# huggingface/tokenizers

Hardware: NVIDIA H100
Metric: encode_batch input throughput (higher is better)
Workload: dtype u8

## Files before the change

### __graft_entry__.py

```python
import os, subprocess, sys

ROOT = os.path.dirname(os.path.abspath(__file__))
if ROOT not in sys.path:
    sys.path.insert(0, ROOT)


def build():
    subprocess.check_call(["make", "-s", "-C", os.path.join(ROOT, "tokenizers_b200", "csrc")])
    subprocess.check_call(["make", "-s", "-C", os.path.join(ROOT, "oracle")])
    sys.path.insert(0, os.path.join(ROOT, "tools"))
    import corpus
    corpus.build()
    subprocess.check_call(["g++", "-O2", "-std=c++17", "-shared", "-fPIC", "-o", os.path.join(ROOT, "tests", "native", "libpretok_emul.so"),
                           os.path.join(ROOT, "tests", "native", "pretok_emul.cpp")])
    subprocess.check_call(["g++", "-O2", "-std=c++17", "-I/usr/local/cuda/include", "-Wno-attributes", "-shared", "-fPIC", "-o",
                           os.path.join(ROOT, "tests", "native", "libadded_emul.so"), os.path.join(ROOT, "tests", "native", "added_emul.cpp")])
    subprocess.check_call(["g++", "-O2", "-std=c++17", "-I/usr/local/cuda/include", "-Wno-attributes", "-shared", "-fPIC", "-o",
                           os.path.join(ROOT, "tests", "native", "libdense_emul.so"), os.path.join(ROOT, "tests", "native", "dense_emul.cpp")])
    subprocess.check_call(["g++", "-O2", "-std=c++17", "-I/usr/local/cuda/include", "-Wno-attributes", "-shared", "-fPIC", "-o",
                           os.path.join(ROOT, "tests", "native", "liboverflow_emul.so"), os.path.join(ROOT, "tests", "native", "overflow_emul.cpp")])
    subprocess.check_call(["g++", "-O2", "-std=c++17", "-I/usr/local/cuda/include", "-Wno-attributes", "-shared", "-fPIC", "-o",
                           os.path.join(ROOT, "tests", "native", "libmeta_emul.so"), os.path.join(ROOT, "tests", "native", "meta_emul.cpp")])
    subprocess.check_call(["g++", "-O2", "-std=c++17", "-I/usr/local/cuda/include", "-Wno-attributes", "-shared", "-fPIC", "-include", "cuda_runtime.h", "-o",
                           os.path.join(ROOT, "tests", "native", "libnorm_emul.so"), os.path.join(ROOT, "tests", "native", "norm_emul.cpp"),
                           "-x", "c++", os.path.join(ROOT, "tokenizers_b200", "csrc", "host_tables.cu")])
    import tokenizers_b200
    from tokenizers_b200 import _lib
    _lib.lib()


def smoke():
    import gzip
    import numpy as np
    sys.path.insert(0, os.path.join(ROOT, "tools"))
    import corpus
    from tokenizers_b200 import Tokenizer
    from oracle import oracle as orc
    for name, kind in (("gpt2_style", 2), ("llama3_style", 2), ("wordpiece", 4)):
        js = gzip.open(os.path.join(ROOT, "assets", name + ".json.gz")).read().decode("utf-8")
        tok = Tokenizer.from_str(js, device=0)
        data, off = corpus.generate(kind, 7, 0, 2000)
        be = tok.encode_batch_csr(data, off)
        ids, offs, wid, rp = orc.Oracle(js).encode_batch_csr(data, off)
        assert np.array_equal(be.ids, ids) and np.array_equal(be.offsets, offs) and np.array_equal(be.word_ids, wid) and np.array_equal(be.row_ptr, rp), name
        print(f"smoke {name}: {len(off) - 1} docs, {len(data)} bytes -> {len(ids)} tokens, bit-exact vs oracle")
    import json
    j = json.loads(gzip.open(os.path.join(ROOT, "assets", "wordpiece.json.gz")).read().decode("utf-8"))
    j["normalizer"] = {"type": "BertNormalizer", "clean_text": True, "handle_chinese_chars": True, "strip_accents": None, "lowercase": True}
    j["pre_tokenizer"] = {"type": "BertPreTokenizer"}
    js = json.dumps(j)
    tok = Tokenizer.from_str(js, device=0)
    data, off = corpus.generate(2, 8, 0, 1500)
    be = tok.encode_batch_csr(data, off)
    ids, offs, wid, rp = orc.Oracle(js).encode_batch_csr(data, off)
    assert np.array_equal(be.ids, ids) and np.array_equal(be.offsets, offs) and np.array_equal(be.word_ids, wid) and np.array_equal(be.row_ptr, rp), "bert"
    tok.enable_truncation(32); tok.enable_padding(length=32, pad_id=0)
    dn = tok.encode_batch_dense(data, off, add_special_tokens=False)
    exp = orc.dense_rows(ids, rp, length=32, pad_to_multiple_of=0, max_length=32, pad_id=0, truncate_left=False, pad_left=False, pre=[], post=[])
    assert np.array_equal(dn["input_ids"], exp[0]) and np.array_equal(dn["attention_mask"], exp[1]), "dense"
    print(f"smoke bert_uncased: {len(off) - 1} docs -> {len(ids)} tokens, offsets into the original text and dense [n, 32] rows bit-exact vs oracle")


if __name__ == "__main__":
    build()
    if len(sys.argv) > 1 and sys.argv[1] == "smoke":
        smoke()
```

### tokenizers_b200/csrc/b2t_tables.h

```cpp
#pragma once
#include <stdint.h>

#if defined(__CUDACC__)
#define B2T_HDI __host__ __device__ __forceinline__
#else
#define B2T_HDI inline
#endif

namespace b2t {

constexpr uint32_t EMPTY_KEY = 0xFFFFFFFFu;
constexpr uint64_t NO_MERGE = ~0ull;

B2T_HDI uint32_t pair_hash(uint32_t a, uint32_t b) {
  uint32_t h = a * 0x9E3779B1u ^ (b * 0x85EBCA77u + 0x165667B1u);
  h ^= h >> 15; h *= 0x2C1B3C6Du; h ^= h >> 12;
  return h;
}

struct StrHash {
  uint32_t h1, h2;
};
B2T_HDI void strhash_init(StrHash& s) { s.h1 = 0x811C9DC5u; s.h2 = 0x9747B28Cu; }
B2T_HDI void strhash_byte(StrHash& s, uint32_t b) {
  s.h1 = (s.h1 ^ b) * 0x01000193u;
  s.h2 = (s.h2 + b + 1u) * 0x5BD1E995u; s.h2 ^= s.h2 >> 13;
}
B2T_HDI void strhash_fin(StrHash& s) {
  s.h1 ^= s.h1 >> 16; s.h1 *= 0x7FEB352Du; s.h1 ^= s.h1 >> 15;
  s.h2 ^= s.h2 >> 15; s.h2 *= 0x846CA68Bu; s.h2 ^= s.h2 >> 16;
}

B2T_HDI uint32_t edge_hash(uint32_t node, uint32_t byte) {
  uint32_t h = (node * 256u + byte) * 0x9E3779B1u;
  h ^= h >> 16; h *= 0x85EBCA6Bu; h ^= h >> 13;
  return h;
}

enum { NORM_IDENT = 0u, NORM_REMOVE = 1u, NORM_STRING = 2u, NORM_SURVIVOR = 3u, NORM_MARK_FLAG = 4u, NORM_TAIL_FLAG = 0x80u };
constexpr uint32_t NORM_LEN_MASK = 31u;

B2T_HDI bool norm_mark_neighbour(uint32_t cp, uint32_t e, const uint8_t* ascii) {
  if (cp < 128u) return ascii[cp] == 0xFFu;
  const uint32_t kind = e & 3u;
  return kind == NORM_SURVIVOR || (kind == NORM_REMOVE && (e & NORM_MARK_FLAG) != 0u);
}

struct DeviceTables {
  const uint32_t* byte_to_id;
  const uint4* merge_tbl;
  uint32_t merge_mask;
  const uint4* word_tbl;
  uint32_t word_mask;
  const uint8_t* word_pool;
  int ignore_merges;
  int monotone;
  const uint32_t* tok2_bits;
  const uint32_t* tri_bits;
  const uint4* edge_tbl;
  uint32_t edge_mask;
  uint32_t unk_id;
  uint32_t max_chars;
};

}
```

### tokenizers_b200/csrc/engine.cu

```cuda
#include <cuda_runtime.h>
#include <stdarg.h>
#include <stdio.h>
#include <stdlib.h>
#include <string.h>

#include <algorithm>
#include <atomic>
#include <condition_variable>
#include <memory>
#include <mutex>
#include <string>
#include <vector>

#include "../../include/b2t.h"
#include "added_kernels.cuh"
#include "dense_kernels.cuh"
#include "host_tables.h"
#include "long_kernels.cuh"
#include "model_kernels.cuh"
#include "norm_kernels.cuh"
#include "prefix_kernels.cuh"
#include "pretok_kernels.cuh"

using namespace b2t;
// ... 113 lines not shown
  DevBuf bytes, doc_off;
  DevBuf doc_bits, start_bits, drop_bits, page_sum, page_carry, block_sum, block_carry, page_first_doc, ctl;
  DevBuf ids, offsets, word_ids, row_ptr, row_ptr_local;
  Request req;
  Batch batch;
  bool pending = false;
  DevBuf tmp_ids, tmp_offsets, tmp_word_ids, tile_count, tile_first, tile_lexcl, tile_bsum;
  DevBuf page_long, long_desc, long_desc1, soft_bits, page_soft, lp_id, lp_val, lp_len, lp_plen, lp_aux, lp_out;
  unsigned long long pool_cap = 0;
  DevBuf wcache;
  DevBuf dense_ids, dense_mask, dense_len, dense_type;
  DevBuf dense_off, row_count, row_lexcl, row_bsum, row_base, row_sample;
  DevBuf dense_special, dense_seq, dense_word;
  DevBuf nrm_doc_bits, nrm_pfd, nrm_page_out, nrm_page_chars, nrm_lexcl_o, nrm_bsum_o, nrm_lexcl_c, nrm_bsum_c, nrm_tot, nrm_bytes, nrm_src_char, nrm_doc_off, nrm_doc_char0;
  bool norm_active = false;
  DevBuf cand0, cand1, cand_any, hard_bits, inner_bits, added_bits, added_head, added_pool;
  uint32_t added_cap = 0;
  DevBuf pfx_bytes, pfx_doc_off, pfx_local, pfx_block, prefix_bits, pfx_total;
  cudaStream_t stream = nullptr;
  cudaEvent_t done = nullptr;
  PinBuf h_ctl;
  ~Workspace() {
    if (stream) cudaStreamDestroy(stream);
    if (done) cudaEventDestroy(done);
  }
};

struct b2t_result {
  b2t_engine* eng = nullptr;
  int on_device = 0;
  uint32_t n_docs = 0;
  uint64_t n_tokens = 0;
  const uint32_t* ids = nullptr; const uint32_t* offsets = nullptr; const uint32_t* word_ids = nullptr; const uint64_t* row_ptr = nullptr;
  PinBuf h_ids, h_offsets, h_word_ids, h_row_ptr;
  uint32_t dense_len = 0;
  const uint32_t* dense_ids = nullptr; const uint8_t* dense_mask = nullptr; const uint32_t* row_len = nullptr;
  const uint8_t* type_ids = nullptr;
  uint32_t n_rows = 0;
  const uint32_t* row_sample = nullptr; const uint32_t* dense_off = nullptr;
  const uint8_t* special_mask = nullptr; const int8_t* seq_ids = nullptr; const uint32_t* dense_word = nullptr;
  PinBuf h_dense_ids, h_dense_mask, h_row_len, h_type_ids, h_row_sample, h_dense_off, h_special, h_seq, h_word;
};

constexpr int NSLOT = 3;
constexpr int MAX_KERNEL_RECORDS = 16;

struct b2t_engine {
  int device = 0;
  int model = 0, pretok = 0, add_prefix_space = 0;
  int sm_count = 132;
  int wcache_on = 1;
  DeviceTables dt;
  int monotone = 0;
  DevBuf d_cls, d_byte_to_id, d_merge, d_word, d_pool, d_edge, d_tok2, d_tri;
  int norm_on = 0;
  NormTables nt;
  DevBuf d_nt_blk, d_nt_ent, d_nt_pool, d_nt_ascii;
  int has_added = 0;
  AddedTables at;
  DevBuf d_at_bytes, d_at_off, d_at_id, d_at_flags, d_at_first, d_at_pair, d_cls_rust;
  DevBuf d_trim_vocab, d_trim_added;
  uint32_t n_trim_added = 0;
  int trim_ready = 0, added_both = 0;
  std::mutex mu;
  std::mutex dev_mu;
  std::mutex prof_mu;
  std::condition_variable set_free;
  Workspace dev_ws;
  struct SlotSet { Workspace slot[NSLOT]; bool busy = false; };
  std::vector<std::unique_ptr<SlotSet>> sets;
  cudaStream_t own_stream = nullptr;
  size_t chunk_bytes = 64u << 20;
  std::vector<std::unique_ptr<b2t_result>> pool;
  int profiling = 0;
  int n_rec = 0;
  const char* rec_name[MAX_KERNEL_RECORDS];
  cudaEvent_t rec_ev[MAX_KERNEL_RECORDS + 1];
  bool rec_ev_made = false;
  std::atomic<int> last_launches{0};
  ~b2t_engine() {
    if (rec_ev_made) for (auto& ev : rec_ev) cudaEventDestroy(ev);
    if (own_stream) cudaStreamDestroy(own_stream);
  }
};
constexpr size_t MAX_SLOT_SETS = 4;

template <class T>
static int upload(DevBuf& b, const std::vector<T>& v) {
  size_t bytes = v.size() * sizeof(T);
  int rc = b.ensure(bytes ? bytes : 16);
  if (rc) return rc;
  if (bytes) CU(cudaMemcpy(b.p, v.data(), bytes, cudaMemcpyHostToDevice));
  return B2T_OK;
}

extern "C" int b2t_engine_create(const b2t_config* cfg, b2t_engine** out) {
  if (!cfg || !out) return fail(B2T_ERR_INVALID, "b2t_engine_create: null argument");
  if (cfg->struct_size != sizeof(b2t_config)) return fail(B2T_ERR_INVALID, "b2t_engine_create: struct_size mismatch (%u != %zu)", cfg->struct_size, sizeof(b2t_config));
  *out = nullptr;
  if (cfg->model != B2T_MODEL_BPE && cfg->model != B2T_MODEL_WORDPIECE) return fail(B2T_ERR_UNSUPPORTED, "unsupported model kind %d", cfg->model);
  if (cfg->pretok < 0 || cfg->pretok > 4) return fail(B2T_ERR_UNSUPPORTED, "unsupported pre-tokenizer kind %d", cfg->pretok);
  if (cfg->model == B2T_MODEL_BPE && (cfg->pretok == B2T_PRETOK_WHITESPACE || cfg->pretok == B2T_PRETOK_BERT))
    return fail(B2T_ERR_UNSUPPORTED, "BPE is supported behind the ByteLevel pre-tokenizers only");
  if (cfg->model == B2T_MODEL_WORDPIECE && cfg->pretok != B2T_PRETOK_WHITESPACE && cfg->pretok != B2T_PRETOK_BERT)
    return fail(B2T_ERR_UNSUPPORTED, "WordPiece is supported behind the Whitespace and Bert pre-tokenizers only");
  if ((cfg->bert_normalizer & B2T_NORM_BERT) && cfg->model != B2T_MODEL_WORDPIECE)
    return fail(B2T_ERR_UNSUPPORTED, "BertNormalizer is supported in front of WordPiece pipelines only");
  if (cfg->bert_normalizer & ~(B2T_NORM_BERT | B2T_NORM_CLEAN_TEXT | B2T_NORM_CHINESE_CHARS | B2T_NORM_STRIP_ACCENTS | B2T_NORM_LOWERCASE))
    return fail(B2T_ERR_INVALID, "unknown bits in bert_normalizer");
  if (cfg->add_prefix_space && cfg->pretok != B2T_PRETOK_BYTELEVEL && cfg->pretok != B2T_PRETOK_BYTELEVEL_NOREGEX)
    return fail(B2T_ERR_UNSUPPORTED, "add_prefix_space is only meaningful for a top-level ByteLevel pre-tokenizer");
  if (!cfg->vocab_bytes || !cfg->vocab_off || !cfg->vocab_ids || cfg->n_vocab == 0) return fail(B2T_ERR_INVALID, "empty vocabulary");

  HostTables ht;
  bool vocab_err = false;
  std::string msg = build_host_tables(cfg->model, cfg->pretok, cfg->ignore_merges, cfg->n_vocab, cfg->vocab_bytes, cfg->vocab_off,
                                      cfg->vocab_ids, cfg->n_merges, cfg->merge_bytes, cfg->merge_off, cfg->unk_token,
                                      cfg->continuing_subword_prefix, cfg->max_input_chars_per_word, &ht, &vocab_err);
  if (!msg.empty()) return fail(vocab_err ? B2T_ERR_VOCAB : B2T_ERR_UNSUPPORTED, "%s", msg.c_str());

  int ndev = 0;
  cudaError_t ce = cudaGetDeviceCount(&ndev);
  if (ce != cudaSuccess || ndev == 0)
    return fail(B2T_ERR_CUDA, "no CUDA device available (%s); this engine has no CPU path", cudaGetErrorString(ce));
  int dev = cfg->device;
  if (dev < 0) CU(cudaGetDevice(&dev));
  if (dev >= ndev) return fail(B2T_ERR_INVALID, "device %d out of range (%d devices)", dev, ndev);
  CU(cudaSetDevice(dev));

  std::unique_ptr<b2t_engine, void (*)(b2t_engine*)> e(new b2t_engine(), b2t_engine_destroy);
  e->device = dev; e->model = cfg->model; e->pretok = cfg->pretok; e->add_prefix_space = cfg->add_prefix_space;
  cudaDeviceGetAttribute(&e->sm_count, cudaDevAttrMultiProcessorCount, dev);
  if (const char* wc = getenv("B2T_WCACHE")) e->wcache_on = atoi(wc) != 0;
  if (const char* cb = getenv("B2T_CHUNK_BYTES")) {
    long long v = atoll(cb);
    if (v >= 1024 && v < (1ll << 31)) e->chunk_bytes = (size_t)v;
  }
  int rc = B2T_OK;
  if ((rc = upload(e->d_cls, ht.cls_packed)) || (rc = upload(e->d_byte_to_id, ht.byte_to_id)) || (rc = upload(e->d_merge, ht.merge_tbl)) ||
      (rc = upload(e->d_word, ht.word_tbl)) || (rc = upload(e->d_pool, ht.word_pool)) || (rc = upload(e->d_edge, ht.edge_tbl)) ||
      (rc = upload(e->d_tok2, ht.tok2_bits)) || (rc = upload(e->d_tri, ht.tri_bits)))
    return rc;
  if (cfg->bert_normalizer & B2T_NORM_BERT) {
    NormHost nh;
    build_bert_norm((cfg->bert_normalizer & B2T_NORM_CLEAN_TEXT) != 0, (cfg->bert_normalizer & B2T_NORM_CHINESE_CHARS) != 0,
                    (cfg->bert_normalizer & B2T_NORM_STRIP_ACCENTS) != 0, (cfg->bert_normalizer & B2T_NORM_LOWERCASE) != 0, &nh);
    if (!nh.ok) return fail(B2T_ERR_UNSUPPORTED, "BertNormalizer table: an image exceeds three bytes per input byte");
    if ((rc = upload(e->d_nt_blk, nh.blk)) || (rc = upload(e->d_nt_ent, nh.ent)) || (rc = upload(e->d_nt_pool, nh.pool)) || (rc = upload(e->d_nt_ascii, nh.ascii)))
      return rc;
    e->nt.blk = e->d_nt_blk.as<uint16_t>(); e->nt.ent = e->d_nt_ent.as<uint32_t>(); e->nt.pool = e->d_nt_pool.as<uint8_t>(); e->nt.ascii = e->d_nt_ascii.as<uint8_t>();
    e->norm_on = 1;
  }
  memset(&e->dt, 0, sizeof(e->dt));
  e->dt.byte_to_id = e->d_byte_to_id.as<uint32_t>();
  e->dt.merge_tbl = e->d_merge.as<uint4>();
  e->dt.merge_mask = ht.merge_tbl.empty() ? 0 : (uint32_t)ht.merge_tbl.size() - 1;
  e->dt.word_tbl = e->d_word.as<uint4>();
  e->dt.word_mask = ht.word_tbl.empty() ? 0 : (uint32_t)ht.word_tbl.size() - 1;
  e->dt.word_pool = e->d_pool.as<uint8_t>();
  e->dt.ignore_merges = cfg->ignore_merges ? 1 : 0;
  e->dt.monotone = ht.monotone ? 1 : 0;
  e->dt.tok2_bits = e->d_tok2.as<uint32_t>(); e->dt.tri_bits = e->d_tri.as<uint32_t>();
  e->monotone = e->dt.monotone;
  e->dt.edge_tbl = e->d_edge.as<uint4>();
  e->dt.edge_mask = ht.edge_tbl.empty() ? 0 : (uint32_t)ht.edge_tbl.size() - 1;
  e->dt.unk_id = ht.unk_id;
  e->dt.max_chars = ht.max_chars;
  cudaFuncSetAttribute(model_tile_kernel<MODEL_BPE>, cudaFuncAttributePreferredSharedMemoryCarveout, 86);
  cudaFuncSetAttribute(model_tile_kernel<MODEL_WORDPIECE>, cudaFuncAttributePreferredSharedMemoryCarveout, 86);
  if (cfg->model == B2T_MODEL_BPE) {
    if ((rc = upload(e->d_trim_vocab, vocab_trim_counts(cfg->n_vocab, cfg->vocab_bytes, cfg->vocab_off, cfg->vocab_ids)))) return rc;
    e->trim_ready = 1;
  }
  cudaError_t se = cudaStreamCreateWithFlags(&e->own_stream, cudaStreamNonBlocking);
  if (se != cudaSuccess) return fail(B2T_ERR_CUDA, "cudaStreamCreate failed: %s", cudaGetErrorString(se));
  *out = e.release();
  return B2T_OK;
}

extern "C" void b2t_engine_destroy(b2t_engine* e) {
  if (!e) return;
  cudaSetDevice(e->device);
  cudaDeviceSynchronize();
  delete e;
}

struct ctl_block {
  uint32_t max_row;
  uint32_t err;
  unsigned long long total;
  LongCtl lc;
  uint32_t added_used;
  uint32_t max_all;
  unsigned long long rows;
  uint32_t stride_m;
  uint32_t pad;
};

static int ensure_long_pool(Workspace& ws, unsigned long long bytes) {
  if (bytes <= ws.pool_cap) return B2T_OK;
  unsigned long long cap = bytes + bytes / 4 + 4096;
  int rc;
  if ((rc = ws.lp_id.ensure(cap * 4)) || (rc = ws.lp_val.ensure(cap * 8)) || (rc = ws.lp_len.ensure(cap * 4)) || (rc = ws.lp_plen.ensure(cap * 4)) ||
      (rc = ws.lp_aux.ensure(cap * 4)) || (rc = ws.lp_out.ensure(cap * 16)))
    return rc;
  ws.pool_cap = cap;
  return B2T_OK;
}

template <int KIND>
static void launch_pretok(b2t_engine* e, const uint8_t* d_bytes, int64_t n, Workspace& ws, cudaStream_t st, bool added) {
  const int64_t n_chunks = n / CHUNK + 1;
  const int64_t n_kb = (n_chunks + 31) / 32;
  const int64_t resident = (int64_t)e->sm_count * (KIND == PT_LLAMA3 ? K1_WINDOW_MINBLOCKS : K1_LEAN_MINBLOCKS) * (K1_THREADS / 32);
  int64_t kb = (n_kb + resident * 4 - 1) / (resident * 4);
  kb = std::min<int64_t>(128, std::max<int64_t>(2, (kb + 1) & ~1ll));
  const int64_t n_warps = (n_kb + kb - 1) / kb;
  const int64_t grid = (n_warps + (K1_THREADS / 32) - 1) / (K1_THREADS / 32);
// ... 1137 lines not shown
```

### tokenizers_b200/csrc/host_tables.cu

```cuda
#include "host_tables.h"

#include <string.h>
#include <vector_types.h>

#include <algorithm>

#include "pretok_logic.cuh"
#include "unicode_ranges.inc"
#include "bert_tables.inc"

namespace b2t {

void unicode_class_table(int scheme, uint8_t* out) {
  memset(out, 0, 0x110000);
  auto fill = [&](const uint32_t (*r)[2], uint32_t cnt, uint8_t v) {
    for (uint32_t i = 0; i < cnt; ++i)
      for (uint32_t c = r[i][0]; c <= r[i][1]; ++c) out[c] = v;
  };
  if (scheme == 0) {
    fill(B2T_ONIG_L, B2T_ONIG_L_COUNT, CLS_L);
    fill(B2T_ONIG_N, B2T_ONIG_N_COUNT, CLS_N);
    fill(B2T_ONIG_S, B2T_ONIG_S_COUNT, CLS_S);
  } else if (scheme == 2) {
    memset(out, CLS_L, 0x110000);
// ... 83 lines not shown
            if (!in_ranges(B2T_BERT_MN, B2T_BERT_MN_COUNT, x)) {
              seq.push_back(x);
              kept_mark = kept_mark || in_ranges(B2T_BERT_CCC, B2T_BERT_CCC_COUNT, x);
            }
        }
        if (lowercase) {
          tmp.clear();
          for (uint32_t x : seq) { auto it = low.find(x); if (it == low.end()) tmp.push_back(x); else tmp.insert(tmp.end(), it->second.begin(), it->second.end()); }
          seq.swap(tmp);
        }
        const bool reorders = strip_accents && in_ranges(B2T_BERT_CCC, B2T_BERT_CCC_COUNT, c);
        if (seq.empty()) e = NORM_REMOVE | (reorders || (strip_accents && cleaned) ? NORM_MARK_FLAG : 0u);
        else if (reorders) {
          e = (seq.size() == 1 && seq[0] == c) ? NORM_SURVIVOR : (NORM_SURVIVOR | NORM_MARK_FLAG);
        } else if (!(seq.size() == 1 && seq[0] == c)) {
          img.clear();
          for (uint32_t x : seq) utf8_append(img, x);
          const size_t src_len = c < 0x80 ? 1 : (c < 0x800 ? 2 : (c < 0x10000 ? 3 : 4));
          if (img.size() > 3 * src_len || img.size() > NORM_LEN_MASK) out->ok = false;
          e = NORM_STRING | ((uint32_t)img.size() << 2) | ((uint32_t)out->pool.size() << 8) | (kept_mark ? NORM_TAIL_FLAG : 0u);
          out->pool.insert(out->pool.end(), img.begin(), img.end());
        }
        if (c < 128) out->ascii[c] = seq.empty() ? 0xFF : (uint8_t)seq[0];
      }
      block[c - b0] = e;
      any = any || e != NORM_IDENT;
    }
    if (any) { out->blk[b0 >> 7] = (uint16_t)(out->ent.size() / 128); out->ent.insert(out->ent.end(), block.begin(), block.end()); }
  }
  out->pool.resize(out->pool.size() + 16, 0);
}

static void utf8_append(std::string& s, uint32_t cp) {
  if (cp < 0x80) s.push_back((char)cp);
  else if (cp < 0x800) { s.push_back((char)(0xC0 | (cp >> 6))); s.push_back((char)(0x80 | (cp & 63))); }
  else if (cp < 0x10000) { s.push_back((char)(0xE0 | (cp >> 12))); s.push_back((char)(0x80 | ((cp >> 6) & 63))); s.push_back((char)(0x80 | (cp & 63))); }
  else { s.push_back((char)(0xF0 | (cp >> 18))); s.push_back((char)(0x80 | ((cp >> 12) & 63))); s.push_back((char)(0x80 | ((cp >> 6) & 63))); s.push_back((char)(0x80 | (cp & 63))); }
}

static void bytes_char_table(uint32_t cp_of_byte[256]) {
  uint32_t k = 0;
  for (int b = 0; b < 256; ++b) {
    bool printable = (b >= '!' && b <= '~') || (b >= 0xA1 && b <= 0xAC) || (b >= 0xAE && b <= 0xFF);
    cp_of_byte[b] = printable ? (uint32_t)b : 256u + k++;
  }
}

static uint32_t pow2_at_least(uint64_t x) {
  uint32_t c = 16;
  while (c < x) c <<= 1;
  return c;
}

std::string build_host_tables(int model, int pretok, int ignore_merges, uint32_t n_vocab, const uint8_t* vocab_bytes,
                              const uint32_t* vocab_off, const uint32_t* vocab_ids, uint32_t n_merges,
                              const uint8_t* merge_bytes, const uint32_t* merge_off, const char* unk_token,
                              const char* cont_prefix, uint32_t max_chars, HostTables* out, bool* vocab_err) {
  *vocab_err = false;
  {
    std::vector<uint8_t> cls(0x110000);
    unicode_class_table(pretok == PT_BERT ? 2 : (pretok == PT_WHITESPACE ? 1 : 0), cls.data());
    out->cls_packed.assign(0x110000 / 16, 0u);
    for (uint32_t c = 0; c < 0x110000; ++c) out->cls_packed[c >> 4] |= (uint32_t)cls[c] << ((c & 15) * 2);
  }
  std::unordered_map<std::string, uint32_t> vocab;
  vocab.reserve((size_t)n_vocab * 2);
  for (uint32_t i = 0; i < n_vocab; ++i) {
    if (vocab_ids[i] >= (1u << 20)) return "token ids of 2^20 and above are not supported";
    vocab[std::string((const char*)vocab_bytes + vocab_off[i], vocab_off[i + 1] - vocab_off[i])] = vocab_ids[i];
  }
  out->max_chars = max_chars;

  if (model == 0) {
    uint32_t cp_of_byte[256];
    bytes_char_table(cp_of_byte);
    std::unordered_map<uint32_t, uint8_t> byte_of_cp;
    out->byte_to_id.assign(256, 0);
    for (int b = 0; b < 256; ++b) {
      std::string ch;
      utf8_append(ch, cp_of_byte[b]);
      auto it = vocab.find(ch);
      if (it == vocab.end())
        return "BPE vocab lacks the ByteLevel character of byte " + std::to_string(b) +
               " (the reference would silently drop such bytes; unsupported on device)";
      out->byte_to_id[b] = it->second;
      byte_of_cp[cp_of_byte[b]] = (uint8_t)b;
    }
    uint32_t cap = pow2_at_least((uint64_t)n_merges * 5 / 2 + 16);
    out->merge_tbl.assign(cap, make_uint4(EMPTY_KEY, EMPTY_KEY, EMPTY_KEY, EMPTY_KEY));
    for (uint32_t i = 0; i < n_merges; ++i) {
      std::string a((const char*)merge_bytes + merge_off[2 * i], merge_off[2 * i + 1] - merge_off[2 * i]);
      std::string b((const char*)merge_bytes + merge_off[2 * i + 1], merge_off[2 * i + 2] - merge_off[2 * i + 1]);
      auto ia = vocab.find(a), ib = vocab.find(b), in = vocab.find(a + b);
      if (ia == vocab.end() || ib == vocab.end() || in == vocab.end()) {
        *vocab_err = true;
        return "merge " + std::to_string(i) + ": token out of vocabulary";
      }
      uint32_t h = pair_hash(ia->second, ib->second) & (cap - 1);
      while (true) {
        uint4& e = out->merge_tbl[h];
        if (e.x == EMPTY_KEY || (e.x == ia->second && e.y == ib->second)) {
          e = make_uint4(ia->second, ib->second, i, in->second);
          break;
        }
        h = (h + 1) & (cap - 1);
      }
    }
    {
      std::unordered_map<uint32_t, uint32_t> created;
      bool mono = true;
      uint32_t live = 0;
      for (const uint4& e : out->merge_tbl) {
        if (e.x == EMPTY_KEY) continue;
        ++live;
        auto it = created.find(e.w);
        if (it == created.end() || it->second < e.z) created[e.w] = e.z;
      }
      if (live != n_merges) mono = false;
      for (const uint4& e : out->merge_tbl) {
        if (e.x == EMPTY_KEY) continue;
        auto ia = created.find(e.x), ib = created.find(e.y);
        if ((ia != created.end() && ia->second >= e.z) || (ib != created.end() && ib->second >= e.z)) { mono = false; break; }
      }
      out->monotone = mono;
    }
    {
      out->tok2_bits.assign((1u << 16) / 32, 0u);
      out->tri_bits.assign((1u << 24) / 32, 0u);
      for (uint32_t i = 0; i < n_vocab; ++i) {
        const uint8_t* s = vocab_bytes + vocab_off[i];
        const uint32_t len = vocab_off[i + 1] - vocab_off[i];
        std::vector<uint8_t> raw;
        bool ok = len > 0;
        for (uint32_t p = 0; p < len && ok;) {
          uint32_t b0 = s[p], cp, l;
          if (b0 < 0x80) { cp = b0; l = 1; }
          else if (b0 < 0xE0 && p + 1 < len) { cp = ((b0 & 31u) << 6) | (s[p + 1] & 63u); l = 2; }
          else { ok = false; break; }
          auto it = byte_of_cp.find(cp);
          if (it == byte_of_cp.end()) { ok = false; break; }
          raw.push_back((uint8_t)it->second);
          p += l;
        }
        if (!ok) continue;
        if (raw.size() == 2) { const uint32_t k = raw[0] | ((uint32_t)raw[1] << 8); out->tok2_bits[k >> 5] |= 1u << (k & 31); }
        for (size_t p = 0; p + 2 < raw.size(); ++p) {
          const uint32_t k = raw[p] | ((uint32_t)raw[p + 1] << 8) | ((uint32_t)raw[p + 2] << 16);
          out->tri_bits[k >> 5] |= 1u << (k & 31);
        }
      }
    }
    if (ignore_merges) {
      uint32_t wcap = pow2_at_least((uint64_t)n_vocab * 5 / 2 + 16);
      out->word_tbl.assign(wcap, make_uint4(0, 0, EMPTY_KEY, 0));
      for (uint32_t i = 0; i < n_vocab; ++i) {
        const uint8_t* s = vocab_bytes + vocab_off[i];
        uint32_t len = vocab_off[i + 1] - vocab_off[i];
        std::string raw;
        bool ok = len > 0;
        for (uint32_t p = 0; p < len && ok;) {
          uint32_t b0 = s[p], cp, l;
          if (b0 < 0x80) { cp = b0; l = 1; }
          else if (b0 < 0xE0 && p + 1 < len) { cp = ((b0 & 31u) << 6) | (s[p + 1] & 63u); l = 2; }
          else { ok = false; break; }
          auto it = byte_of_cp.find(cp);
          if (it == byte_of_cp.end()) { ok = false; break; }
          raw.push_back((char)it->second);
          p += l;
        }
        if (!ok) continue;
        StrHash h;
        strhash_init(h);
        for (unsigned char c : raw) strhash_byte(h, c);
        strhash_fin(h);
        uint32_t slot = h.h1 & (wcap - 1);
        while (out->word_tbl[slot].z != EMPTY_KEY) slot = (slot + 1) & (wcap - 1);
        out->word_tbl[slot] = make_uint4(h.h2, (uint32_t)raw.size(), vocab_ids[i], (uint32_t)out->word_pool.size());
        out->word_pool.insert(out->word_pool.end(), raw.begin(), raw.end());
      }
      out->word_pool.resize(out->word_pool.size() + 16, 0);
    }
  } else {
    if (!unk_token) return "WordPiece needs unk_token";
    if ((uint64_t)max_chars * 4 > 416) return "max_input_chars_per_word above 104 is not supported";
    auto iu = vocab.find(unk_token);
    if (iu == vocab.end()) {
      *vocab_err = true;
      return "WordPiece error: Missing [UNK] token from the vocabulary";
    }
    out->unk_id = iu->second;
    std::string prefix = cont_prefix ? cont_prefix : "";
    std::unordered_map<uint64_t, uint32_t> edges;
    std::vector<uint32_t> node_tok(2, EMPTY_KEY);
    auto insert = [&](uint32_t root, const uint8_t* s, uint32_t len, uint32_t id) {
      uint32_t node = root;
      for (uint32_t p = 0; p < len; ++p) {
        uint64_t key = ((uint64_t)node << 8) | s[p];
        auto it = edges.find(key);
        if (it == edges.end()) {
          uint32_t child = (uint32_t)node_tok.size();
          node_tok.push_back(EMPTY_KEY);
          edges.emplace(key, child);
          node = child;
        } else node = it->second;
      }
      node_tok[node] = id;
    };
    for (uint32_t i = 0; i < n_vocab; ++i) {
      const uint8_t* s = vocab_bytes + vocab_off[i];
      uint32_t len = vocab_off[i + 1] - vocab_off[i];
      if (len == 0) continue;
      insert(0, s, len, vocab_ids[i]);
      if (len > prefix.size() && memcmp(s, prefix.data(), prefix.size()) == 0)
        insert(1, s + prefix.size(), len - (uint32_t)prefix.size(), vocab_ids[i]);
    }
    if (node_tok.size() >= (1u << 24)) return "WordPiece vocabulary too large for the device trie";
    uint32_t ecap = pow2_at_least((uint64_t)edges.size() * 5 / 2 + 16);
    out->edge_tbl.assign(ecap, make_uint4(EMPTY_KEY, 0, EMPTY_KEY, 0));
    for (auto& kv : edges) {
      uint32_t node = (uint32_t)(kv.first >> 8), byte = (uint32_t)(kv.first & 255);
      uint32_t slot = edge_hash(node, byte) & (ecap - 1);
      while (out->edge_tbl[slot].x != EMPTY_KEY) slot = (slot + 1) & (ecap - 1);
      out->edge_tbl[slot] = make_uint4((uint32_t)kv.first, kv.second, node_tok[kv.second], 0);
    }
  }
  return "";
}

}
```

### tokenizers_b200/csrc/host_tables.h

```cpp
#pragma once
#include <stdint.h>
#include <string>
#include <unordered_map>
#include <vector>
#include "b2t_tables.h"

namespace b2t {

struct HostTables {
  std::vector<uint32_t> cls_packed;
  std::vector<uint32_t> byte_to_id;
  std::vector<uint4> merge_tbl;
  std::vector<uint4> word_tbl;
  std::vector<uint8_t> word_pool;
  std::vector<uint4> edge_tbl;
  std::vector<uint32_t> tok2_bits;
  std::vector<uint32_t> tri_bits;
  uint32_t unk_id = EMPTY_KEY;
  uint32_t max_chars = 100;
  bool monotone = false;
};

struct NormHost {
  std::vector<uint16_t> blk;
  std::vector<uint32_t> ent;
  std::vector<uint8_t> pool;
  std::vector<uint8_t> ascii;
  bool ok = true;
};
void build_bert_norm(bool clean_text, bool handle_chinese_chars, bool strip_accents, bool lowercase, NormHost* out);

void unicode_class_table(int scheme, uint8_t* out);

void space_counts(const uint8_t* s, uint32_t len, const uint8_t* cls, uint32_t* chars, uint32_t* lead, uint32_t* trail);

std::vector<uint32_t> vocab_trim_counts(uint32_t n_vocab, const uint8_t* vocab_bytes, const uint32_t* vocab_off, const uint32_t* vocab_ids);

std::string build_host_tables(int model, int pretok, int ignore_merges, uint32_t n_vocab, const uint8_t* vocab_bytes,
                              const uint32_t* vocab_off, const uint32_t* vocab_ids, uint32_t n_merges,
                              const uint8_t* merge_bytes, const uint32_t* merge_off, const char* unk_token,
                              const char* cont_prefix, uint32_t max_chars, HostTables* out, bool* vocab_err);

}
```

### tokenizers_b200/csrc/model_kernels.cuh

```cuda
#pragma once
#include <cuda_runtime.h>
#include <stdint.h>
#include <type_traits>
#include "b2t_tables.h"
#include "added_kernels.cuh"
#include "long_kernels.cuh"
#include "pretok_logic.cuh"

namespace b2t {

constexpr int TILE = PAGE;
constexpr int MODEL_THREADS = 256;
constexpr int THREAD_PATH_MAX = 32;
enum { MODEL_BPE = 0, MODEL_WORDPIECE = 1 };
enum { F_OFFSETS = 1u, F_WORD_IDS = 2u, F_BYTE_OFFSETS = 4u };
constexpr int MAX_LONG_PER_PAGE = TILE / (LONG_PRETOK_MIN + 1) + 1;

struct ModelParams {
  const uint8_t* bytes; int64_t n;
  const uint32_t* start_bits; const uint32_t* drop_bits; const uint32_t* doc_bits;
  const uint32_t* soft_bits; const uint8_t* page_soft;
  const uint64_t* page_carry; const uint64_t* block_carry; const uint32_t* page_first_doc;
  const uint64_t* doc_off; uint32_t n_docs;
  uint32_t flags;
  uint32_t* ids; uint32_t* offsets; uint32_t* word_ids; uint64_t* row_ptr;
  uint32_t* tile_count; uint32_t* tile_first; uint32_t* err_flag;
  int64_t n_tiles;
  const int32_t* page_long; const LongDesc* long_desc; const uint4* long_out;
  uint4* wcache; uint32_t wcache_mask; int wcache_on;
  const uint32_t* prefix_bits;
  const uint32_t* added_bits; const uint32_t* added_head; const uint2* added_pool; uint32_t flag_added;
  DeviceTables t;
};

__device__ __forceinline__ uint64_t merge_lookup(const DeviceTables& t, uint32_t a, uint32_t b) {
  const uint32_t hf = pair_hash(a, b);
  uint32_t h = hf & t.merge_mask;
  while (true) {
    uint4 e = __ldg(t.merge_tbl + h);
    if (e.x == a && e.y == b) return ((uint64_t)e.z << 32) | e.w;
    if (e.x == EMPTY_KEY) return NO_MERGE;
    h = (h + 1) & t.merge_mask;
  }
}

__device__ __forceinline__ int warp_prefix_words(const uint32_t* bits, uint16_t* pref, int nw, int lane) {
  int c0 = 0, c1 = 0, c2 = 0;
  int i = lane * 3;
  if (i < nw) c0 = __popc(bits[i]);
  if (i + 1 < nw) c1 = __popc(bits[i + 1]);
  if (i + 2 < nw) c2 = __popc(bits[i + 2]);
  int tot = c0 + c1 + c2, inc = tot;
#pragma unroll
  for (int s = 1; s < 32; s <<= 1) {
    int o = __shfl_up_sync(0xFFFFFFFFu, inc, s);
    if (lane >= s) inc += o;
  }
  int ex = inc - tot;
  if (i < nw) pref[i] = (uint16_t)ex;
  if (i + 1 < nw) pref[i + 1] = (uint16_t)(ex + c0);
  if (i + 2 < nw) pref[i + 2] = (uint16_t)(ex + c0 + c1);
  return __shfl_sync(0xFFFFFFFFu, inc, 31);
}

__device__ __forceinline__ uint32_t mask_le(int b) { return b >= 31 ? 0xFFFFFFFFu : ((2u << b) - 1u); }

constexpr int TOK_ID_BITS = 20;
__device__ __forceinline__ uint32_t tok_pack(uint32_t id, int len) { return id | ((uint32_t)len << TOK_ID_BITS); }
__device__ __forceinline__ int tok_len(uint32_t x) { return (int)(x >> TOK_ID_BITS); }
__device__ __forceinline__ uint32_t tok_id(uint32_t x) { return x & ((1u << TOK_ID_BITS) - 1u); }


constexpr int WC_MAX_BYTES = 24, WC_MAX_TOK = 6, WC_PROBES = 4;
constexpr int P4_SPLIT_BYTES = 16;
constexpr int P4_SHORT_G = 8;
#define B2T_WC_READY (1ull << 63)
#define B2T_WC_BUSY (1ull << 62)
#define B2T_WC_FP ((1ull << 62) - 1ull)

struct WordKey {
  uint32_t k[6];
  uint32_t slot;
  unsigned long long fp;
};

__device__ __forceinline__ void wc_make_key(const uint8_t* s_byte, int s, int len, WordKey& key) {
  const uint32_t* w = reinterpret_cast<const uint32_t*>(s_byte) + (s >> 2);
  const uint32_t sh = (uint32_t)(s & 3) * 8u;
  uint32_t a0 = w[0], a1 = w[1], a2 = w[2], a3 = w[3], a4 = w[4], a5 = w[5], a6 = w[6];
  uint32_t k[6] = {__funnelshift_r(a0, a1, sh), __funnelshift_r(a1, a2, sh), __funnelshift_r(a2, a3, sh),
                   __funnelshift_r(a3, a4, sh), __funnelshift_r(a4, a5, sh), __funnelshift_r(a5, a6, sh)};
#pragma unroll
  for (int i = 0; i < 6; ++i) {
    const int v = min(len - 4 * i, 4);
    const uint32_t m = __funnelshift_rc(0xFFFFFFFFu, 0u, (uint32_t)(32 - 8 * v));
    key.k[i] = k[i] & m;
  }
  uint32_t a = key.k[0] ^ (key.k[2] * 0x9E3779B1u) ^ (key.k[4] * 0x85EBCA77u);
  uint32_t b = key.k[1] ^ (key.k[3] * 0xC2B2AE3Du) ^ (key.k[5] * 0x27D4EB2Fu);
  a = (a ^ (uint32_t)len) * 0x2C1B3C6Du; b = (b + a) * 0x297A2D39u;
  a ^= b >> 15; a *= 0x85EBCA6Bu; b ^= a >> 13; b *= 0xC2B2AE35u; a ^= b >> 16;
  key.slot = a;
  key.fp = ((((unsigned long long)b << 32) | a) ^ ((unsigned long long)len << 56)) & B2T_WC_FP;
  if (key.fp == 0) key.fp = 1;
}

__device__ __forceinline__ uint4 ld_relaxed_v4(const uint4* p) {
  uint4 v;
  asm volatile("ld.relaxed.gpu.global.v4.u32 {%0, %1, %2, %3}, [%4];" : "=r"(v.x), "=r"(v.y), "=r"(v.z), "=r"(v.w) : "l"(p) : "memory");
  return v;
}
__device__ __forceinline__ void st_relaxed_v4(uint4* p, uint4 v) {
  asm volatile("st.relaxed.gpu.global.v4.u32 [%0], {%1, %2, %3, %4};" ::"l"(p), "r"(v.x), "r"(v.y), "r"(v.z), "r"(v.w) : "memory");
}
constexpr uint32_t WC_LEN_MARK = 0x80000000u;

__device__ __forceinline__ bool wc_lookup(const ModelParams& P, const uint8_t* s_byte, uint32_t* s_tok, int s, int len, bool skip) {
  if (!P.wcache_on || len > WC_MAX_BYTES || skip) return false;
  WordKey key;
  wc_make_key(s_byte, s, len, key);
  const uint4* cache = P.wcache;
  const uint32_t mask = P.wcache_mask;
  uint32_t slot = key.slot & mask;
#pragma unroll 1
  for (int pr = 0; pr < WC_PROBES; ++pr, slot = (slot + 1) & mask) {
    const uint4* q = cache + (size_t)slot * 4;
    const uint4 q0 = ld_relaxed_v4(q);
    const unsigned long long tag = ((unsigned long long)q0.y << 32) | q0.x;
    if (tag == 0ull) return false;
    if (tag != (B2T_WC_READY | key.fp)) {
      if (tag == (B2T_WC_BUSY | key.fp)) return false;
      continue;
    }
    if (q0.z != ~key.k[0] || q0.w != ~key.k[1]) continue;
    const uint4 q1 = ld_relaxed_v4(q + 1);
    if (q1.x != ~key.k[2] || q1.y != ~key.k[3] || q1.z != ~key.k[4] || q1.w != ~key.k[5]) continue;
    const uint4 q2 = ld_relaxed_v4(q + 2);
    const int ntok = (int)(q2.x & 0xFFu);
    const uint4 q3 = ntok > 2 ? ld_relaxed_v4(q + 3) : make_uint4(0u, 0u, 0u, 0u);
    const uint32_t cids[6] = {q2.z, q2.w, q3.x, q3.y, q3.z, q3.w};
    const uint32_t lens[6] = {(q2.x >> 8) & 0xFFu, (q2.x >> 16) & 0xFFu, q2.x >> 24, q2.y & 0xFFu, (q2.y >> 8) & 0xFFu, (q2.y >> 16) & 0xFFu};
    bool ok = ntok != 0 && (q2.y & WC_LEN_MARK);
#pragma unroll
    for (int t = 0; t < WC_MAX_TOK; ++t) ok = ok && (t >= ntok || cids[t] != 0u);
    if (!ok) return false;
    int pos = s;
#pragma unroll
    for (int t = 0; t < WC_MAX_TOK; ++t)
      if (t < ntok) { s_tok[pos] = tok_pack(~cids[t], (int)lens[t]); pos += (int)lens[t]; }
    return true;
  }
  return false;
}

__device__ __forceinline__ void wc_publish(const ModelParams& P, const uint8_t* s_byte, const uint32_t* s_tok, int s, int e, bool skip) {
  if (!P.wcache_on || e - s > WC_MAX_BYTES || skip) return;
  WordKey key;
  wc_make_key(s_byte, s, e - s, key);
  uint4* const cache = P.wcache;
  const uint32_t mask = P.wcache_mask;
  uint32_t ids[6] = {0, 0, 0, 0, 0, 0}, lens[6] = {0, 0, 0, 0, 0, 0};
  int nt = 0, p = s;
  while (p < e) {
    if (nt == WC_MAX_TOK) return;
    const uint32_t tk = s_tok[p];
    const int l = tok_len(tk);
#pragma unroll
    for (int t = 0; t < WC_MAX_TOK; ++t) if (t == nt) { ids[t] = tok_id(tk); lens[t] = (uint32_t)l; }
    ++nt; p += l;
  }
  uint32_t slot = key.slot & mask;
#pragma unroll 1
  for (int pr = 0; pr < WC_PROBES; ++pr, slot = (slot + 1) & mask) {
// ... 685 lines not shown
```

Before: 55.42.

## Add read-only whole-word vocabulary table probed before the word cache

Builds a host-side hash table of vocabulary entries up to 12 bytes whose BPE merges reduce to the token itself (or any entry for WordPiece), and uploads it to the device. The word-cache lookup first probes this static table, so common whole-word tokens resolve with read-only loads instead of running the merge loop or going through the atomic word cache. This adds table-build time on the host, extra device memory, and one extra probe per short word that misses.

```diff
diff --git a/__graft_entry__.py b/__graft_entry__.py
--- a/__graft_entry__.py
+++ b/__graft_entry__.py
@@ -23,6 +23,9 @@
                            os.path.join(ROOT, "tests", "native", "libmeta_emul.so"), os.path.join(ROOT, "tests", "native", "meta_emul.cpp")])
     subprocess.check_call(["g++", "-O2", "-std=c++17", "-I/usr/local/cuda/include", "-Wno-attributes", "-shared", "-fPIC", "-include", "cuda_runtime.h", "-o",
                            os.path.join(ROOT, "tests", "native", "libnorm_emul.so"), os.path.join(ROOT, "tests", "native", "norm_emul.cpp"),
+                           "-x", "c++", os.path.join(ROOT, "tokenizers_b200", "csrc", "host_tables.cu")])
+    subprocess.check_call(["g++", "-O2", "-std=c++17", "-I/usr/local/cuda/include", "-Wno-attributes", "-shared", "-fPIC", "-include", "cuda_runtime.h", "-o",
+                           os.path.join(ROOT, "tests", "native", "libvocab_table_emul.so"), os.path.join(ROOT, "tests", "native", "vocab_table_emul.cpp"),
                            "-x", "c++", os.path.join(ROOT, "tokenizers_b200", "csrc", "host_tables.cu")])
     import tokenizers_b200
     from tokenizers_b200 import _lib
diff --git a/tokenizers_b200/csrc/b2t_tables.h b/tokenizers_b200/csrc/b2t_tables.h
--- a/tokenizers_b200/csrc/b2t_tables.h
+++ b/tokenizers_b200/csrc/b2t_tables.h
@@ -31,6 +31,42 @@
   s.h2 ^= s.h2 >> 15; s.h2 *= 0x846CA68Bu; s.h2 ^= s.h2 >> 16;
 }
 
+struct WordHash {
+  uint32_t a, b;
+};
+B2T_HDI WordHash word_key_hash(const uint32_t k[6], uint32_t len) {
+  uint32_t a = k[0] ^ (k[2] * 0x9E3779B1u) ^ (k[4] * 0x85EBCA77u);
+  uint32_t b = k[1] ^ (k[3] * 0xC2B2AE3Du) ^ (k[5] * 0x27D4EB2Fu);
+  a = (a ^ len) * 0x2C1B3C6Du; b = (b + a) * 0x297A2D39u;
+  a ^= b >> 15; a *= 0x85EBCA6Bu; b ^= a >> 13; b *= 0xC2B2AE35u; a ^= b >> 16;
+  return {a, b};
+}
+
+constexpr int TOK_ID_BITS = 20;
+B2T_HDI uint32_t tok_pack(uint32_t id, int len) { return id | ((uint32_t)len << TOK_ID_BITS); }
+B2T_HDI int tok_len(uint32_t x) { return (int)(x >> TOK_ID_BITS); }
+B2T_HDI uint32_t tok_id(uint32_t x) { return x & ((1u << TOK_ID_BITS) - 1u); }
+
+constexpr int VOCAB_KEY_BYTES = 12;
+constexpr int VOCAB_LOAD_SHIFT = 2;
+B2T_HDI uint4 ld_readonly(const uint4* p) {
+#if defined(__CUDA_ARCH__)
+  return __ldg(p);
+#else
+  return *p;
+#endif
+}
+B2T_HDI uint32_t vocab_probe(const uint4* tbl, uint32_t mask, uint32_t probes, const uint32_t k[6], int len, uint32_t a) {
+  uint32_t slot = a & mask;
+#pragma unroll 1
+  for (uint32_t pr = 0; pr <= probes; ++pr, slot = (slot + 1) & mask) {
+    const uint4 e = ld_readonly(tbl + slot);
+    if (e.w == 0u) return 0u;
+    if (e.x == k[0] && e.y == k[1] && e.z == k[2] && tok_len(e.w) == len) return e.w;
+  }
+  return 0u;
+}
+
 B2T_HDI uint32_t edge_hash(uint32_t node, uint32_t byte) {
   uint32_t h = (node * 256u + byte) * 0x9E3779B1u;
   h ^= h >> 16; h *= 0x85EBCA6Bu; h ^= h >> 13;
@@ -57,6 +93,9 @@
   int monotone;
   const uint32_t* tok2_bits;
   const uint32_t* tri_bits;
+  const uint4* vocab_tbl;
+  uint32_t vocab_mask;
+  uint32_t vocab_probes;
   const uint4* edge_tbl;
   uint32_t edge_mask;
   uint32_t unk_id;
diff --git a/tokenizers_b200/csrc/engine.cu b/tokenizers_b200/csrc/engine.cu
--- a/tokenizers_b200/csrc/engine.cu
+++ b/tokenizers_b200/csrc/engine.cu
@@ -189,7 +189,7 @@
   int wcache_on = 1;
   DeviceTables dt;
   int monotone = 0;
-  DevBuf d_cls, d_byte_to_id, d_merge, d_word, d_pool, d_edge, d_tok2, d_tri;
+  DevBuf d_cls, d_byte_to_id, d_merge, d_word, d_pool, d_edge, d_tok2, d_tri, d_vocab;
   int norm_on = 0;
   NormTables nt;
   DevBuf d_nt_blk, d_nt_ent, d_nt_pool, d_nt_ascii;
@@ -276,7 +276,7 @@
   int rc = B2T_OK;
   if ((rc = upload(e->d_cls, ht.cls_packed)) || (rc = upload(e->d_byte_to_id, ht.byte_to_id)) || (rc = upload(e->d_merge, ht.merge_tbl)) ||
       (rc = upload(e->d_word, ht.word_tbl)) || (rc = upload(e->d_pool, ht.word_pool)) || (rc = upload(e->d_edge, ht.edge_tbl)) ||
-      (rc = upload(e->d_tok2, ht.tok2_bits)) || (rc = upload(e->d_tri, ht.tri_bits)))
+      (rc = upload(e->d_tok2, ht.tok2_bits)) || (rc = upload(e->d_tri, ht.tri_bits)) || (rc = upload(e->d_vocab, ht.vocab_tbl)))
     return rc;
   if (cfg->bert_normalizer & B2T_NORM_BERT) {
     NormHost nh;
@@ -301,6 +301,9 @@
   e->monotone = e->dt.monotone;
   e->dt.edge_tbl = e->d_edge.as<uint4>();
   e->dt.edge_mask = ht.edge_tbl.empty() ? 0 : (uint32_t)ht.edge_tbl.size() - 1;
+  e->dt.vocab_tbl = e->d_vocab.as<uint4>();
+  e->dt.vocab_mask = (uint32_t)ht.vocab_tbl.size() - 1;
+  e->dt.vocab_probes = ht.vocab_probes;
   e->dt.unk_id = ht.unk_id;
   e->dt.max_chars = ht.max_chars;
   cudaFuncSetAttribute(model_tile_kernel<MODEL_BPE>, cudaFuncAttributePreferredSharedMemoryCarveout, 86);
diff --git a/tokenizers_b200/csrc/host_tables.cu b/tokenizers_b200/csrc/host_tables.cu
--- a/tokenizers_b200/csrc/host_tables.cu
+++ b/tokenizers_b200/csrc/host_tables.cu
@@ -159,6 +159,60 @@
   return c;
 }
 
+static bool byte_level_raw(const uint8_t* s, uint32_t len, const uint8_t byte_of_cp[512], const bool in_alphabet[512], std::string* raw) {
+  raw->clear();
+  for (uint32_t p = 0; p < len;) {
+    uint32_t b0 = s[p], cp, l;
+    if (b0 < 0x80) { cp = b0; l = 1; }
+    else if (b0 < 0xE0 && p + 1 < len) { cp = ((b0 & 31u) << 6) | (s[p + 1] & 63u); l = 2; }
+    else return false;
+    if (cp >= 512 || !in_alphabet[cp]) return false;
+    raw->push_back((char)byte_of_cp[cp]);
+    p += l;
+  }
+  return len > 0;
+}
+
+static void build_vocab_table(const std::vector<std::pair<std::string, uint32_t>>& entries, HostTables* out) {
+  const uint32_t cap = pow2_at_least((uint64_t)entries.size() << VOCAB_LOAD_SHIFT);
+  out->vocab_tbl.assign(cap, make_uint4(0u, 0u, 0u, 0u));
+  out->vocab_probes = 0;
+  for (const auto& en : entries) {
+    uint32_t k[6] = {0, 0, 0, 0, 0, 0};
+    for (size_t i = 0; i < en.first.size(); ++i) k[i >> 2] |= (uint32_t)(uint8_t)en.first[i] << (8 * (i & 3));
+    const uint32_t len = (uint32_t)en.first.size();
+    uint32_t slot = word_key_hash(k, len).a & (cap - 1), dist = 0;
+    while (out->vocab_tbl[slot].w != 0u) { slot = (slot + 1) & (cap - 1); ++dist; }
+    out->vocab_tbl[slot] = make_uint4(k[0], k[1], k[2], tok_pack(en.second, (int)len));
+    out->vocab_probes = std::max(out->vocab_probes, dist);
+  }
+}
+
+static uint32_t merge_to_one(const std::string& raw, const HostTables& ht) {
+  std::vector<uint32_t> sym(raw.size());
+  for (size_t i = 0; i < raw.size(); ++i) sym[i] = ht.byte_to_id[(uint8_t)raw[i]];
+  const uint32_t mask = (uint32_t)ht.merge_tbl.size() - 1;
+  auto lookup = [&](uint32_t a, uint32_t b) -> const uint4* {
+    for (uint32_t h = pair_hash(a, b) & mask;; h = (h + 1) & mask) {
+      const uint4& e = ht.merge_tbl[h];
+      if (e.x == a && e.y == b) return &e;
+      if (e.x == EMPTY_KEY) return nullptr;
+    }
+  };
+  while (sym.size() > 1) {
+    size_t best = 0;
+    const uint4* bm = nullptr;
+    for (size_t i = 0; i + 1 < sym.size(); ++i) {
+      const uint4* m = lookup(sym[i], sym[i + 1]);
+      if (m && (!bm || m->z < bm->z)) { bm = m; best = i; }
+    }
+    if (!bm) break;
+    sym[best] = bm->w;
+    sym.erase(sym.begin() + best + 1);
+  }
+  return sym.size() == 1 ? sym[0] : EMPTY_KEY;
+}
+
 std::string build_host_tables(int model, int pretok, int ignore_merges, uint32_t n_vocab, const uint8_t* vocab_bytes,
                               const uint32_t* vocab_off, const uint32_t* vocab_ids, uint32_t n_merges,
                               const uint8_t* merge_bytes, const uint32_t* merge_off, const char* unk_token,
@@ -181,7 +235,8 @@
   if (model == 0) {
     uint32_t cp_of_byte[256];
     bytes_char_table(cp_of_byte);
-    std::unordered_map<uint32_t, uint8_t> byte_of_cp;
+    uint8_t byte_of_cp[512] = {};
+    bool in_alphabet[512] = {};
     out->byte_to_id.assign(256, 0);
     for (int b = 0; b < 256; ++b) {
       std::string ch;
@@ -191,8 +246,12 @@
         return "BPE vocab lacks the ByteLevel character of byte " + std::to_string(b) +
                " (the reference would silently drop such bytes; unsupported on device)";
       out->byte_to_id[b] = it->second;
-      byte_of_cp[cp_of_byte[b]] = (uint8_t)b;
-    }
+      byte_of_cp[cp_of_byte[b]] = (uint8_t)b; in_alphabet[cp_of_byte[b]] = true;
+    }
+    std::vector<std::string> raw(n_vocab);
+    std::vector<uint8_t> ok(n_vocab);
+    for (uint32_t i = 0; i < n_vocab; ++i)
+      ok[i] = byte_level_raw(vocab_bytes + vocab_off[i], vocab_off[i + 1] - vocab_off[i], byte_of_cp, in_alphabet, &raw[i]);
     uint32_t cap = pow2_at_least((uint64_t)n_merges * 5 / 2 + 16);
     out->merge_tbl.assign(cap, make_uint4(EMPTY_KEY, EMPTY_KEY, EMPTY_KEY, EMPTY_KEY));
     for (uint32_t i = 0; i < n_merges; ++i) {
@@ -235,24 +294,11 @@
       out->tok2_bits.assign((1u << 16) / 32, 0u);
       out->tri_bits.assign((1u << 24) / 32, 0u);
       for (uint32_t i = 0; i < n_vocab; ++i) {
-        const uint8_t* s = vocab_bytes + vocab_off[i];
-        const uint32_t len = vocab_off[i + 1] - vocab_off[i];
-        std::vector<uint8_t> raw;
-        bool ok = len > 0;
-        for (uint32_t p = 0; p < len && ok;) {
-          uint32_t b0 = s[p], cp, l;
-          if (b0 < 0x80) { cp = b0; l = 1; }
-          else if (b0 < 0xE0 && p + 1 < len) { cp = ((b0 & 31u) << 6) | (s[p + 1] & 63u); l = 2; }
-          else { ok = false; break; }
-          auto it = byte_of_cp.find(cp);
-          if (it == byte_of_cp.end()) { ok = false; break; }
-          raw.push_back((uint8_t)it->second);
-          p += l;
-        }
-        if (!ok) continue;
-        if (raw.size() == 2) { const uint32_t k = raw[0] | ((uint32_t)raw[1] << 8); out->tok2_bits[k >> 5] |= 1u << (k & 31); }
-        for (size_t p = 0; p + 2 < raw.size(); ++p) {
-          const uint32_t k = raw[p] | ((uint32_t)raw[p + 1] << 8) | ((uint32_t)raw[p + 2] << 16);
+        if (!ok[i]) continue;
+        const uint8_t* r = reinterpret_cast<const uint8_t*>(raw[i].data());
+        if (raw[i].size() == 2) { const uint32_t k = r[0] | ((uint32_t)r[1] << 8); out->tok2_bits[k >> 5] |= 1u << (k & 31); }
+        for (size_t p = 0; p + 2 < raw[i].size(); ++p) {
+          const uint32_t k = r[p] | ((uint32_t)r[p + 1] << 8) | ((uint32_t)r[p + 2] << 16);
           out->tri_bits[k >> 5] |= 1u << (k & 31);
         }
       }
@@ -261,31 +307,24 @@
       uint32_t wcap = pow2_at_least((uint64_t)n_vocab * 5 / 2 + 16);
       out->word_tbl.assign(wcap, make_uint4(0, 0, EMPTY_KEY, 0));
       for (uint32_t i = 0; i < n_vocab; ++i) {
-        const uint8_t* s = vocab_bytes + vocab_off[i];
-        uint32_t len = vocab_off[i + 1] - vocab_off[i];
-        std::string raw;
-        bool ok = len > 0;
-        for (uint32_t p = 0; p < len && ok;) {
-          uint32_t b0 = s[p], cp, l;
-          if (b0 < 0x80) { cp = b0; l = 1; }
-          else if (b0 < 0xE0 && p + 1 < len) { cp = ((b0 & 31u) << 6) | (s[p + 1] & 63u); l = 2; }
-          else { ok = false; break; }
-          auto it = byte_of_cp.find(cp);
-          if (it == byte_of_cp.end()) { ok = false; break; }
-          raw.push_back((char)it->second);
-          p += l;
-        }
-        if (!ok) continue;
+        if (!ok[i]) continue;
         StrHash h;
         strhash_init(h);
-        for (unsigned char c : raw) strhash_byte(h, c);
+        for (unsigned char c : raw[i]) strhash_byte(h, c);
         strhash_fin(h);
         uint32_t slot = h.h1 & (wcap - 1);
         while (out->word_tbl[slot].z != EMPTY_KEY) slot = (slot + 1) & (wcap - 1);
-        out->word_tbl[slot] = make_uint4(h.h2, (uint32_t)raw.size(), vocab_ids[i], (uint32_t)out->word_pool.size());
-        out->word_pool.insert(out->word_pool.end(), raw.begin(), raw.end());
+        out->word_tbl[slot] = make_uint4(h.h2, (uint32_t)raw[i].size(), vocab_ids[i], (uint32_t)out->word_pool.size());
+        out->word_pool.insert(out->word_pool.end(), raw[i].begin(), raw[i].end());
       }
       out->word_pool.resize(out->word_pool.size() + 16, 0);
+    }
+    {
+      std::vector<std::pair<std::string, uint32_t>> entries;
+      for (uint32_t i = 0; i < n_vocab; ++i)
+        if (ok[i] && raw[i].size() <= (size_t)VOCAB_KEY_BYTES && (ignore_merges || merge_to_one(raw[i], *out) == vocab_ids[i]))
+          entries.emplace_back(raw[i], vocab_ids[i]);
+      build_vocab_table(entries, out);
     }
   } else {
     if (!unk_token) return "WordPiece needs unk_token";
@@ -330,6 +369,14 @@
       while (out->edge_tbl[slot].x != EMPTY_KEY) slot = (slot + 1) & (ecap - 1);
       out->edge_tbl[slot] = make_uint4((uint32_t)kv.first, kv.second, node_tok[kv.second], 0);
     }
+    std::vector<std::pair<std::string, uint32_t>> entries;
+    for (const auto& kv : vocab) {
+      uint32_t chars = 0;
+      for (unsigned char c : kv.first) chars += (c & 0xC0u) != 0x80u;
+      if (!kv.first.empty() && kv.first.size() <= (size_t)VOCAB_KEY_BYTES && chars <= max_chars) entries.emplace_back(kv.first, kv.second);
+    }
+    std::sort(entries.begin(), entries.end());
+    build_vocab_table(entries, out);
   }
   return "";
 }
diff --git a/tokenizers_b200/csrc/host_tables.h b/tokenizers_b200/csrc/host_tables.h
--- a/tokenizers_b200/csrc/host_tables.h
+++ b/tokenizers_b200/csrc/host_tables.h
@@ -14,6 +14,8 @@
   std::vector<uint4> word_tbl;
   std::vector<uint8_t> word_pool;
   std::vector<uint4> edge_tbl;
+  std::vector<uint4> vocab_tbl;
+  uint32_t vocab_probes = 0;
   std::vector<uint32_t> tok2_bits;
   std::vector<uint32_t> tri_bits;
   uint32_t unk_id = EMPTY_KEY;
diff --git a/tokenizers_b200/csrc/model_kernels.cuh b/tokenizers_b200/csrc/model_kernels.cuh
--- a/tokenizers_b200/csrc/model_kernels.cuh
+++ b/tokenizers_b200/csrc/model_kernels.cuh
@@ -65,13 +65,10 @@
 
 __device__ __forceinline__ uint32_t mask_le(int b) { return b >= 31 ? 0xFFFFFFFFu : ((2u << b) - 1u); }
 
-constexpr int TOK_ID_BITS = 20;
-__device__ __forceinline__ uint32_t tok_pack(uint32_t id, int len) { return id | ((uint32_t)len << TOK_ID_BITS); }
-__device__ __forceinline__ int tok_len(uint32_t x) { return (int)(x >> TOK_ID_BITS); }
-__device__ __forceinline__ uint32_t tok_id(uint32_t x) { return x & ((1u << TOK_ID_BITS) - 1u); }
 
 
 constexpr int WC_MAX_BYTES = 24, WC_MAX_TOK = 6, WC_PROBES = 4;
+static_assert(VOCAB_KEY_BYTES <= WC_MAX_BYTES, "the vocabulary table keys are word-cache keys");
 constexpr int P4_SPLIT_BYTES = 16;
 constexpr int P4_SHORT_G = 8;
 #define B2T_WC_READY (1ull << 63)
@@ -96,12 +93,9 @@
     const uint32_t m = __funnelshift_rc(0xFFFFFFFFu, 0u, (uint32_t)(32 - 8 * v));
     key.k[i] = k[i] & m;
   }
-  uint32_t a = key.k[0] ^ (key.k[2] * 0x9E3779B1u) ^ (key.k[4] * 0x85EBCA77u);
-  uint32_t b = key.k[1] ^ (key.k[3] * 0xC2B2AE3Du) ^ (key.k[5] * 0x27D4EB2Fu);
-  a = (a ^ (uint32_t)len) * 0x2C1B3C6Du; b = (b + a) * 0x297A2D39u;
-  a ^= b >> 15; a *= 0x85EBCA6Bu; b ^= a >> 13; b *= 0xC2B2AE35u; a ^= b >> 16;
-  key.slot = a;
-  key.fp = ((((unsigned long long)b << 32) | a) ^ ((unsigned long long)len << 56)) & B2T_WC_FP;
+  const WordHash h = word_key_hash(key.k, (uint32_t)len);
+  key.slot = h.a;
+  key.fp = ((((unsigned long long)h.b << 32) | h.a) ^ ((unsigned long long)len << 56)) & B2T_WC_FP;
   if (key.fp == 0) key.fp = 1;
 }
 
@@ -119,6 +113,10 @@
   if (!P.wcache_on || len > WC_MAX_BYTES || skip) return false;
   WordKey key;
   wc_make_key(s_byte, s, len, key);
+  if (len <= VOCAB_KEY_BYTES) {
+    const uint32_t whole = vocab_probe(P.t.vocab_tbl, P.t.vocab_mask, P.t.vocab_probes, key.k, len, key.slot);
+    if (whole) { s_tok[s] = whole; return true; }
+  }
   const uint4* cache = P.wcache;
   const uint32_t mask = P.wcache_mask;
   uint32_t slot = key.slot & mask;
```

Measured after the change: 56.44 (median of 6 runs). 1.8% higher.
